# kalakris/stomp_motion_planner_icra2011

Measured on AMD Instinct MI355X. Metric: STOMP iterations/sec (7-DOF, 100 wp, K=512, 256³ SDF) at 1/2/4/8 GPUs, higher is better.
Workload: dtype f64; 1 GPU; cfg2: 7-DOF, 100 wp (N=99), K=512 (512/GPU), K_r=0, 256^3 SDF, S=49 spheres; global_rollouts=512, rollouts_per_gpu=512, parallelism=rollout shard x1

## Files before the change

### stomp_motion_planner_icra2011_amd/csrc/engine.cpp

```cpp
#include "stomp_engine.h"

#include <hip/hip_runtime.h>

#include <algorithm>
#include <chrono>
#include <cmath>
#include <condition_variable>
#include <map>
#include <memory>
#include <mutex>
#include <cstdarg>
#include <cstdio>
#include <cstdlib>
#include <cstring>
#include <string>
#include <thread>
#include <unordered_map>
#include <vector>

#include "kernels.h"
#include "setup.h"

#ifdef STOMP_WITH_RCCL
#include <rccl/rccl.h>
// ... 72 lines not shown
    SetupOutput su;
    DevModel model{};
    TermsModel terms{};
    bool terms_on = false;
    double* d_terms_traj = nullptr;
    uint8_t* d_cs = nullptr;
    DevTrack* d_track = nullptr;
    const int* d_stop = nullptr;
    double* d_opt_costs = nullptr;
    DevTrack* h_track = nullptr;
    bool tracking = false;
    std::vector<FkOp> ops;
    std::vector<int> sphere_slot;
    int nslots = 0;
    std::vector<void*> allocs;
    double *d_theta = nullptr, *d_LT = nullptr, *d_MT = nullptr, *d_QT = nullptr;
    double *d_params = nullptr, *d_noise = nullptr, *d_control = nullptr, *d_prob = nullptr, *d_state = nullptr;
    double *d_params_b = nullptr, *d_noise_b = nullptr, *d_control_b = nullptr, *d_state_b = nullptr;
    int row_set = 0;
    double *d_cum = nullptr, *d_u = nullptr;
    double *d_x_params = nullptr, *d_x_noise = nullptr, *d_x_control = nullptr, *d_x_state = nullptr;
    double *d_last_traj = nullptr, *d_best_traj = nullptr, *d_total = nullptr;
    double *d_pad_pos = nullptr, *d_start = nullptr, *d_goal = nullptr;
    double *d_tot_loc = nullptr, *d_tot_all = nullptr, *d_tot_x = nullptr, *d_slot = nullptr, *d_slot_all = nullptr;
    double* d_reuse_costs = nullptr;
    int* d_reuse_count = nullptr;
    double *d_spec_params = nullptr, *d_spec_noise = nullptr, *d_spec_ctl = nullptr;
    bool spec_on = false;
    bool pick_fuse = true;
    int* d_sel = nullptr;
// ... 319 lines not shown
    const double co0 = cof(1, 1, 2, 2), co1 = cof(1, 2, 2, 0), co2 = cof(1, 0, 2, 1);
    const double det = M[0] * co0 + M[1] * co1 + M[2] * co2;
    const double sc = 1.0 / det;
    O[0] = co0 * sc; O[1] = cof(0, 2, 2, 1) * sc; O[2] = cof(0, 1, 1, 2) * sc;
    O[3] = co1 * sc; O[4] = cof(0, 0, 2, 2) * sc; O[5] = cof(0, 2, 1, 0) * sc;
    O[6] = co2 * sc; O[7] = cof(0, 1, 2, 0) * sc; O[8] = cof(0, 0, 1, 1) * sc;
}

void release(stomp_engine* e)
{
    if (!e) return;
    if (e->stream) hipStreamSynchronize(e->stream);
    for (auto& v : e->evs) { hipEventDestroy(v.a); hipEventDestroy(v.b); }
    for (auto ev : e->pool) hipEventDestroy(ev);
    for (void* p : e->allocs) hipFree(p);
    if (e->h_total) hipHostFree(e->h_total);
    if (e->h_cf) hipHostFree(e->h_cf);
    if (e->h_track) hipHostFree(e->h_track);
    if (e->h_stall) hipHostFree(e->h_stall);
    for (auto& r : e->coll_ring)
        if (r.ev) hipEventDestroy(r.ev);
#ifdef STOMP_WITH_RCCL
    if (e->comm) ncclCommDestroy(e->comm);
#endif
    if (e->ev_ready) hipEventDestroy(e->ev_ready);
    if (e->ev_done) hipEventDestroy(e->ev_done);
    if (e->own_stream && e->stream) hipStreamDestroy(e->stream);
}

void launch_rollouts(stomp_engine* e, const CostArgs& ca)
{
    DevModel& m = e->model;
    const int nro = ca.num_noisy + (ca.x_params ? 1 : 0);
    if (m.lean && m.nsaves > 0 && nro > m.sv_rows) {
        void* q = nullptr;
        if (hipMalloc(&q, sizeof(double) * (size_t)nro * m.nsaves * 12 * m.N) == hipSuccess) {
            e->allocs.push_back(q);
            m.sv_glob = (double*)q;
            m.sv_rows = nro;
        } else {
            (void)hipGetLastError();
            m.lean = 0;
        }
    }
    launch_cost(m, ca, e->stream);
}

void launch_terms_for(stomp_engine* e, const CostArgs& ca, uint8_t* cs = nullptr)
{
    if (!e->terms_on) return;
    Timed tm(e, T_TERMS);
    TermsArgs ta{};
    ta.stop = e->d_stop;
    ta.traj = ca.traj_out; ta.state = ca.state_out; ta.total = ca.total_out; ta.num_noisy = ca.num_noisy;
    ta.cs = cs;
    if (ca.x_params) {
        ta.x_traj = ca.x_traj; ta.x_state = ca.x_state; ta.x_total = ca.x_total; ta.x_cs = e->d_cs;
// ... 949 lines not shown
            int best = per_cu_full;
            for (int lv = 1; lv <= 2; ++lv)
                if (per_cu[lv] > best) {
                    best = per_cu[lv];
                    m.lean = lv;
                }
        }
        if (const char* v = getenv("STOMP_DEBUG_LEAN")) {
            const int lv = atoi(v);
            if (lv >= 0 && lv <= 2 && rollout_lean_allowed(m, lv)) m.lean = lv;
        }
        if (getenv("STOMP_DEBUG_LEAN_PRINT"))
            fprintf(stderr, "stomp: rollout LDS full %zu / lean1 %zu / lean2 %zu B, workgroups per CU %d / %d / %d, "
                            "needed %d, layout lean %d\n", lds, rollout_lds_bytes(m, 0, 1) + stat,
                    rollout_lds_bytes(m, 0, 2) + stat, per_cu[0], per_cu[1], per_cu[2], need, m.lean);
    }
    if (!cost_supported(m)) CREATE_TRY(fail(e, STOMP_E_UNSUPPORTED, "FK program too large (%d ops, %d segments)",
                                            m.nops, m.nseg));
    {
        const RolloutLds L = rollout_lds(J, N, e->S, m.sph_chunk, m.nsaves, m.nseg, m.nops, m.nslots, 1);
        std::vector<unsigned char> img(L.total - L.sph, 0);
        auto put = [&](size_t off, const void* src, size_t bytes) {
            if (bytes) std::memcpy(img.data() + (off - L.sph), src, bytes);
        };
        std::vector<double> jlim(2 * (size_t)J);
        for (int j = 0; j < J; ++j) { jlim[2 * j] = jmin[j]; jlim[2 * j + 1] = jmax[j]; }
        put(L.sph, sph.data(), sizeof(DevSphere) * e->S);
        put(L.seg, segs.data(), sizeof(DevSegment) * segs.size());
        put(L.ops, e->ops.data(), sizeof(FkOp) * e->ops.size());
        put(L.slot, slot_sph.data(), sizeof(int) * slot_sph.size());
// ... 43 lines not shown
    m.ny_d = (double)m.ny; m.nz_d = (double)m.nz;
    m.hi_x = m.nx - 1.5; m.hi_y = m.ny - 1.5; m.hi_z = m.nz - 1.5;
    m.ox = d->grid.origin[0]; m.oy = d->grid.origin[1]; m.oz = d->grid.origin[2]; m.res = d->grid.resolution;
    m.inv_res = 1.0 / d->grid.resolution;
    m.start = e->d_start; m.goal = e->d_goal;
    const double invTime = 1.0 / e->disc;
    for (int k = 0; k < 7; ++k) {
        m.vel_coef[k] = invTime * kDiffRules[0][k];
        if ((k < kVelTap0 || k > kVelTap1) && kDiffRules[0][k] != 0.0)
            CREATE_TRY(fail(e, STOMP_E_UNSUPPORTED, "velocity rule tap %d outside the kernel's stencil", k));
    }
    m.w_obs = e->w_obs; m.w_con = e->w_con; m.w_tq = e->w_tq;
    m.QT = e->d_QT;
    m.split_cap = std::max(e->K_loc + 2, m.cus / 2 + 1);
    CREATE_TRY(dev_alloc(e, &m.split_cnt, (size_t)m.split_cap));
    if (m.lean && m.nsaves > 0) {
        m.sv_rows = e->K_loc + 1;
        CREATE_TRY(dev_alloc(e, &m.sv_glob, (size_t)m.sv_rows * m.nsaves * 12 * N));
    }
    {
        const char* env = std::getenv("STOMP_DEBUG_SPLIT_MAX");
        m.split_max = env ? std::atoi(env) : 0;
        const char* xi = std::getenv("STOMP_DEBUG_XCTL_INLINE");
        m.x_ctl_inline = xi && std::strcmp(xi, "1") == 0 ? 1 : 0;
    }
    if (getenv("STOMP_DEBUG_LEAN_PRINT")) {
        const int nro = e->K_loc + 1, extra = e->pre_on ? e->rows : 0;
        const int P = rollout_split_pieces(m, nro, extra, false);
        const char* body = P ? "split" : nro <= m.cus ? (m.phased_lds > 0 ? "phased" : "wide")
                                                      : (m.lean ? "lean slot loop" : "slot loop");
        fprintf(stderr, "stomp: model J %d N %d S %d nseg %d nops %d nsaves %d sincos_pre %d sph_chunk %d lean %d "
                        "pregen %d fused_noise %d brick %d, launch of %d rollouts: %s, %d pieces\n",
                J, N, e->S, m.nseg, m.nops, m.nsaves, m.sincos_pre, m.sph_chunk, m.lean, e->pre_on ? 1 : 0,
                J <= 16 ? 1 : 0, m.brick, nro, body, P);
    }
    m.pad_collision = 0;
    launch_pad_fk(m, e->d_start, e->d_goal, e->d_pad_pos, e->d_pad_cf, e->stream);
    int pad_cf = 0;
    if (hipMemcpyAsync(&pad_cf, e->d_pad_cf, sizeof(int), hipMemcpyDeviceToHost, e->stream) != hipSuccess ||
        hipStreamSynchronize(e->stream) != hipSuccess)
        CREATE_TRY(fail(e, STOMP_E_DEVICE, "padding FK failed: %s", hipGetErrorString(hipGetLastError())));
    m.pad_collision = pad_cf;
    e->pad_collision = pad_cf;
    if (hipMemcpyAsync(e->d_last_traj, e->d_theta, sizeof(double) * J * N, hipMemcpyDeviceToDevice, e->stream) !=
            hipSuccess ||
        hipMemcpyAsync(e->d_best_traj, e->d_theta, sizeof(double) * J * N, hipMemcpyDeviceToDevice, e->stream) !=
            hipSuccess)
        CREATE_TRY(fail(e, STOMP_E_DEVICE, "trajectory copies failed"));

// ... 1392 lines not shown
```

### stomp_motion_planner_icra2011_amd/csrc/k_cost.hip

```cpp
#include <algorithm>
#include <cassert>
#include <cstdlib>

#include "device_fk.h"
#include "limits_device.h"
#include "noise_device.h"
#include "stamps.h"

namespace stomp {

namespace {
constexpr int kMaxOps = 64;
constexpr int kMaxSeg = 64;
#ifndef ROLLOUT_BLOCK
#define ROLLOUT_BLOCK 256
#endif
constexpr int kBlock = ROLLOUT_BLOCK;
#ifndef ROLLOUT_MIN_WAVES
#define ROLLOUT_MIN_WAVES (ROLLOUT_BLOCK > 256 ? 4 : 3)
#endif
#ifndef ROLLOUT_WIDE_BLOCK
#define ROLLOUT_WIDE_BLOCK 512
#endif
constexpr int kWideBlock = ROLLOUT_WIDE_BLOCK;
// ... 101 lines not shown
    case 10: STOMP_FOLD_STEP(9) [[fallthrough]];
    case 9: STOMP_FOLD_STEP(8) [[fallthrough]];
    case 8: STOMP_FOLD_STEP(7) [[fallthrough]];
    case 7: STOMP_FOLD_STEP(6) [[fallthrough]];
    case 6: STOMP_FOLD_STEP(5) [[fallthrough]];
    case 5: STOMP_FOLD_STEP(4) [[fallthrough]];
    case 4: STOMP_FOLD_STEP(3) [[fallthrough]];
    case 3: STOMP_FOLD_STEP(2) [[fallthrough]];
    case 2: STOMP_FOLD_STEP(1) [[fallthrough]];
    case 1: STOMP_FOLD_STEP(0) break;
    default: break;
    }
#undef STOMP_FOLD_STEP
}

__device__ __forceinline__ double sphere_speed(const DevModel& m, const double* fb, const double* pad,
                                               const DevSphere& sp, int s, int t)
{
    const int N = m.N;
    double y[7][3];
#pragma unroll
    for (int kk = kVelTap0; kk <= kVelTap1; ++kk) {
        const int tt = t + kk - 3;
        double yf[3];
        apply_lds(fb, N, min(max(tt, 0), N - 1), sp.pos, yf);
        const int row = tt < 0 ? tt + 6 : (tt >= N ? tt - N + 6 : 0);
        const double* src = pad + (row * m.S + s) * 3;
        const bool in = tt >= 0 && tt < N;
#pragma unroll
        for (int c = 0; c < 3; ++c) y[kk][c] = in ? yf[c] : src[c];
    }
    double v0 = 0.0, v1 = 0.0, v2 = 0.0;
#pragma unroll
    for (int kk = kVelTap0; kk <= kVelTap1; ++kk) {
        const double c = m.vel_coef[kk];
        if (c == 0.0) continue;
        v0 += c * y[kk][0];
        v1 += c * y[kk][1];
        v2 += c * y[kk][2];
    }
    return sqrt(v0 * v0 + v1 * v1 + v2 * v2);
}

// ... 113 lines not shown
        for (int u = 0; u < 4; ++u) v[u] = a.x_params[min(idx0 + tid + u * BLOCK, J * N - 1)];
#pragma unroll
        for (int u = 0; u < 4; ++u) {
            const int idx = idx0 + tid + u * BLOCK;
            if (idx < J * N) {
                a.x_prm[idx] = v[u];
                a.x_nse[idx] = 0.0;
                const int d = idx / N, i = idx - d * N;
                zA[d * Nall + i + 6] = v[u] + 0.0;
            }
        }
    }
    rollout_control<BLOCK>(a.nz, 0, zA, zB, tid, a.x_ctl);
}

template <int BLOCK, bool BRICK, bool PHASED = false, bool FK_OVERLAP = true, int LEAN = 0>
__device__ __forceinline__ void rollout_body(const DevModel& m, const CostArgs& a, const int bid)
{
    static_assert(!LEAN || (!PHASED && FK_OVERLAP), "the lean layout is the slot loop's");
    extern __shared__ __attribute__((aligned(16))) unsigned char lds_raw[];
    __shared__ int flag;
    __shared__ int nz_count;
    const int J = m.J, N = m.N, S = m.S;
    const RolloutLds L = rollout_lds(J, N, S, m.sph_chunk, m.nsaves, m.nseg, m.nops, m.nslots, LEAN ? 0 : m.pad_lds,
                                     PHASED, LEAN);
    {
        const int nro = a.num_noisy + (a.x_params ? 1 : 0);
        if (bid >= nro) {
            const int r = bid - nro;
            if (r >= a.pre_rows) {
                totals_block<BLOCK>(a, J, N, r - a.pre_rows, (double*)(lds_raw + L.nzA));
                return;
            }
            const bool own = PHASED && r >= a.row0 && r < a.row0 + a.num_noisy;
            pregen_block<BLOCK>(a, r, own, (double*)(lds_raw + L.nzA), (double*)(lds_raw + L.nzB));
            return;
        }
    }
    if (a.pre_rows > 0 || a.tot_rows > 0) __builtin_amdgcn_s_setprio(2);
    if (a.stop && *a.stop) return;
    double* traj = (double*)(lds_raw + L.traj);
    double* fb = (double*)(lds_raw + L.fb);
    double* sv = LEAN ? global_ptr(m.sv_glob) + (size_t)bid * m.nsaves * 12 * N : (double*)(lds_raw + L.sv);
    double* av = (double*)(lds_raw + L.av);
    unsigned short* nzl = (unsigned short*)(lds_raw + L.nzl);
    const unsigned char* gimg = (const unsigned char*)m.img;
    const DevSphere* sph = (const DevSphere*)(lds_raw + L.sph);
    const DevSegment* seg_s = (const DevSegment*)(lds_raw + L.seg);
    const FkOp* ops_s = (const FkOp*)(lds_raw + L.ops);
    const int* hl_s = (const int*)(lds_raw + L.hl);
    const double* jlim_s = (const double*)(lds_raw + L.jlim);
    CSphere* csph = (CSphere*)gimg;
    CSegment* cseg = (CSegment*)(gimg + (L.seg - L.sph));
    COp* cops = (COp*)(gimg + (L.ops - L.sph));
    CInt* chl = (CInt*)(gimg + (L.hl - L.sph));
    CDouble* cjlim = (CDouble*)(gimg + (L.jlim - L.sph));
    auto op_at = [&](int i) -> FkOp {
        if constexpr (LEAN != 0) return load_op(cops + i);
        else return ops_s[i];
    };
    const double* pad = !LEAN && m.pad_lds ? (const double*)(lds_raw + L.pad) : m.pad_pos;
    const bool sincos_pre = !LEAN && m.sincos_pre;

    STAMP(0);
    BLOCK_BEGIN();
    const int e = bid, tid = threadIdx.x, lane = tid & 63, wv = tid >> 6;
    constexpr int NW = BLOCK / 64;
    const bool extra = e == a.num_noisy;
    const int member = extra ? a.x_member : a.member;
    double* zA = (double*)(lds_raw + L.nzA);
    double* zB = (double*)(lds_raw + L.nzB);
    const bool gen = a.fused_noise == 1 && !extra;
    const bool pre = a.fused_noise == 2 && !extra;
    constexpr int kCopyBatch = 12 * 256 / BLOCK;
    unsigned long long img[kCopyBatch];
    const int nw = LEAN == 0 ? m.img_words : LEAN == 1 ? (int)(S * sizeof(DevSphere) / 8) : 0;
    if constexpr (LEAN != 2) {
#pragma unroll
        for (int u = 0; u < kCopyBatch; ++u) img[u] = m.img[min(tid + u * BLOCK, nw - 1)];
    }
    PreChunk pc0;
    const bool priced = !PHASED && a.ctl_by_pre;
    const int pr = e + a.row0;
    if (pre) {
        if (priced) pre_chunk_load<BLOCK, false>(a.nz, pr, 0, tid, pc0);
        else pre_chunk_load<BLOCK>(a.nz, pr, 0, tid, pc0);
    }
    if (gen) {
        rollout_normals<BLOCK>(a.nz, e, zA, zB, tid);
    } else if (!pre) {
        const double* prm = extra ? a.x_params : a.params + (long long)e * a.stride;
// ... 30 lines not shown
    if (gen) {
        if (defer) rollout_project<BLOCK, true>(a.nz, e, traj, zA, zB, tid);
        else rollout_project<BLOCK>(a.nz, e, traj, zA, zB, tid);
    } else if (pre) {
        if (priced) rollout_from_pre<BLOCK, true, false>(a.nz, pr, e == 0, traj, zA, zB, tid, pc0);
        else if (defer) rollout_from_pre<BLOCK, true>(a.nz, pr, e == 0, traj, zA, zB, tid, pc0);
        else rollout_from_pre<BLOCK>(a.nz, pr, e == 0, traj, zA, zB, tid, pc0);
    }
    if (tid == 0) flag = 0;
    __syncthreads();
    STAMP(1);
    BLOCK_MARK(4);

    {
        __builtin_amdgcn_s_setprio(3);
        if constexpr (LEAN != 0) joint_limit_passes<NW>(m, traj, chl, cjlim, lane, wv);
        else joint_limit_passes<NW>(m, traj, hl_s, jlim_s, lane, wv);
        __builtin_amdgcn_s_setprio(2);
        __syncthreads();
    }
    STAMP(2);
    BLOCK_MARK(5);
    double* tout = extra ? a.x_traj : (a.traj_out ? a.traj_out + (long long)e * J * N : nullptr);
    if (tout)
        for (int idx = tid; idx < J * N; idx += BLOCK) tout[idx] = traj[idx];
    __syncthreads();
    STAMP(3);

    const int t_own = tid - ((N <= 128 && (e & 1)) ? 128 : 0);
    const bool fk_lane = t_own >= 0 && t_own < N;
    const int G = BLOCK / N, pg = tid / N, pt = tid - pg * N;
    Frame C;
    double cum = 0.0, state = 0.0;
    bool col = false;
    auto fk_step = [&](const FkOp& o, const DevSegment& sg) {
        double st = 0.0, ct = 1.0;
        if (sg.q_index >= 0) {
            if (sincos_pre) {
                st = traj[sg.q_index * N + t_own];
                ct = sv[sg.q_index * N + t_own];
            } else {
                det_sincos(traj[sg.q_index * N + t_own], &st, &ct);
            }
        }
        Frame nf;
        if (o.base == kBaseChain) {
            compose(sg, &C, st, ct, nf);
        } else if (o.base == kBaseRoot) {
            compose(sg, nullptr, st, ct, nf);
        } else {
            Frame pf;
            const double* src = sv + (size_t)o.base * 12 * N + t_own;
#pragma unroll
            for (int k = 0; k < 9; ++k) pf.R[k] = src[k * N];
#pragma unroll
            for (int k = 0; k < 3; ++k) pf.p[k] = src[(9 + k) * N];
            compose(sg, &pf, st, ct, nf);
        }
        C = nf;
        if (o.save >= 0) {
            double* dst = sv + (size_t)o.save * 12 * N + t_own;
#pragma unroll
            for (int k = 0; k < 9; ++k) dst[k * N] = C.R[k];
#pragma unroll
            for (int k = 0; k < 3; ++k) dst[(9 + k) * N] = C.p[k];
        }
    };
    auto fk_op = [&](const FkOp& o) {
        if (o.seg < 0 || !fk_lane) return;
        if constexpr (LEAN != 0) {
            const DevSegment sg = load_seg(cseg + o.seg);
            fk_step(o, sg);
        } else {
            fk_step(o, seg_s[o.seg]);
        }
    };
    auto fk_advance = [&](int op) -> int {
        for (; op < m.nops; ++op) {
            const FkOp o = op_at(op);
            fk_op(o);
            if (o.sph_end > o.sph_begin) return op;
        }
        return m.nops;
    };
    if (sincos_pre) {
        const int JN = J * N;
        for (int i0 = tid; i0 - tid < JN; i0 += 3 * BLOCK) {
            double q[3], sn[3], cs[3];
#pragma unroll
            for (int u = 0; u < 3; ++u) q[u] = traj[min(i0 + u * BLOCK, JN - 1)];
#pragma unroll
            for (int u = 0; u < 3; ++u) det_sincos(q[u], &sn[u], &cs[u]);
#pragma unroll
            for (int u = 0; u < 3; ++u) {
                if (i0 + u * BLOCK < JN) {
                    traj[i0 + u * BLOCK] = sn[u];
                    sv[i0 + u * BLOCK] = cs[u];
                }
            }
        }
        __syncthreads();
    }
    if constexpr (PHASED) {
        __builtin_amdgcn_s_setprio(3);
        const int fk_off = t_own - tid;
        const int fk_w0 = -fk_off / 64, fk_w1 = (N - 1 - fk_off) / 64;
        static_assert(!PHASED || BLOCK >= 512, "the phased body prices rows on its non-FK waves");
        if (defer && (wv < fk_w0 || wv > fk_w1)) {
            const int nfk = fk_w1 - fk_w0 + 1;
            const int cw = wv < fk_w0 ? wv : wv - nfk;
            for (int d = cw; d < J; d += NW - nfk)
                wave_control(a.nz, (size_t)pr * J * N, zA, zB, d, lane);
// ... 67 lines not shown
        __syncthreads();
        STAMP(11);
        __builtin_amdgcn_s_setprio(3);
        for (int i = tid; i < nz_count; i += BLOCK) {
            const int it = nzl[i];
            const int qi = it / N, ti = it - qi * N;
            const DevSphere& sp = sph[qi];
            const double pot = potential(sp, sdf_metres(m, (unsigned)av[it]));
            av[it] = pot * sphere_speed(m, fb + (size_t)sp.slot * 12 * N, pad, sp, qi, ti);
        }
        __syncthreads();
        STAMP(12);
        if (fk_lane) fold_avalues(av + t_own, N, S, cum, state);
        __builtin_amdgcn_s_setprio(2);
        STAMP(13);
    } else {
    __builtin_amdgcn_s_setprio(3);
    int op = fk_advance(0);
    __builtin_amdgcn_s_setprio(2);
    int run = 0;
    STAMP(7);
    while (op < m.nops) {
        const FkOp o = op_at(op);
        if (fk_lane) {
#pragma unroll
            for (int k = 0; k < 9; ++k) fb[k * N + t_own] = C.R[k];
#pragma unroll
            for (int k = 0; k < 3; ++k) fb[(9 + k) * N + t_own] = C.p[k];
        }
        if (tid == 0) nz_count = 0;
// ... 25 lines not shown
                    x[i] = F[3 * i] * pos[0] + F[3 * i + 1] * pos[1] + F[3 * i + 2] * pos[2] + F[9 + i];
                bool ok;
                const unsigned idx = sdf_cell<BRICK>(m, x, ok);
                dv[u] = m.sdf[idx];
                okm |= (unsigned)ok << u;
            }
        }
        STAMP(40 + run);
        int next_op = op;
        if constexpr (FK_OVERLAP) {
            __builtin_amdgcn_s_setprio(3);
            next_op = fk_advance(op + 1);
            __builtin_amdgcn_s_setprio(2);
        }
        if (pg < G) {
#pragma unroll
            for (int u = 0; u < kLaneSpheres; ++u) {
                if (u * G >= ns) break;
                const int q = LEAN == 2 ? u : pg + u * G;
                const bool in = q < ns;
                bool nz = false;
                if (in) {
                    int zl, cl;
                    if constexpr (LEAN == 2) {
                        zl = csph[sb + q].zero_lim;
                        cl = csph[sb + q].col_lim;
                    } else {
                        zl = sph[sb + q].zero_lim;
                        cl = sph[sb + q].col_lim;
                    }
                    const int d2 = (okm >> u) & 1u ? (int)dv[u] : 0;
                    col |= d2 < cl;
                    nz = d2 < zl;
                    av[q * N + pt] = nz ? (double)d2 : 0.0;
                }
                const unsigned long long mask = __ballot(nz);
                if (mask) {
                    const int lane_id = tid & 63;
                    const int leader = __ffsll((long long)mask) - 1;
                    int base = 0;
                    if (lane_id == leader) base = atomicAdd(&nz_count, __popcll(mask));
                    base = __shfl(base, leader, 64);
                    if (nz) nzl[base + __popcll(mask & ((1ull << lane_id) - 1ull))] = (unsigned short)(q * N + pt);
                }
            }
        }
        __syncthreads();
        STAMP(11 + 4 * run);
        __builtin_amdgcn_s_setprio(3);
        for (int i = tid; i < nz_count; i += BLOCK) {
            const int it = nzl[i];
            const int qi = it / N, ti = it - qi * N;
            if constexpr (LEAN == 2) {
                const DevSphere sp = load_sph(csph + sb + qi);
                const double pot = potential(sp, sdf_metres(m, (unsigned)av[it]));
                av[it] = pot * sphere_speed(m, fb, pad, sp, sb + qi, ti);
            } else {
                const DevSphere& sp = sph[sb + qi];
// ... 43 lines not shown
            for (; k + 8 <= N; k += 8) {
                double v[8];
#pragma unroll
                for (int q = 0; q < 8; ++q) v[q] = av[k + q];
#pragma unroll
                for (int q = 0; q < 8; ++q) s += v[q];
            }
            for (; k < N; ++k) s += av[k];
            *to = s;
        }
    }
    STAMP(5);
    BLOCK_END();
}

template <int BLOCK, bool BRICK, int LEAN = 0>
__global__ __launch_bounds__(BLOCK, rollout_min_waves<BLOCK>()) void k_rollout(DevModel m, CostArgs a)
{
    rollout_body<BLOCK, BRICK, false, true, LEAN>(m, a, blockIdx.x);
}

template <bool BRICK>
__global__ __launch_bounds__(kWideBlock, kWideBlock > 512 ? 4 : 2) void k_rollout_phased(DevModel m, CostArgs a)
{
    rollout_body<kWideBlock, BRICK, true>(m, a, blockIdx.x);
}

template <int BLOCK, bool BRICK>
__global__ __launch_bounds__(BLOCK, rollout_min_waves<BLOCK>()) void k_rollout_group(const DevModel* ms, const CostArgs* as,
                                                                           int engines, int nro, int npre)
{
    const int b = blockIdx.x;
    int p, bid;
    if (b < engines * nro) {
// ... 464 lines not shown
}

void launch_cost_group(const DevModel& m0, const DevModel* ms, const CostArgs* as, int engines, int nro, int npre,
                       hipStream_t s)
{
    if (engines * (nro + npre) <= 0) return;
    if (m0.brick) launch_cost_group_t<true>(m0, ms, as, engines, nro, npre, s);
    else launch_cost_group_t<false>(m0, ms, as, engines, nro, npre, s);
}

bool cost_supported(const DevModel& m)
{
    return m.nops <= kMaxOps && m.nseg <= kMaxSeg && m.nslots <= kMaxSeg && m.J <= kMaxJoints && m.N <= kBlock;
}

size_t rollout_lds_bytes(const DevModel& m, int pad_lds, int lean)
{
    return rollout_lds(m.J, m.N, m.S, m.sph_chunk, m.nsaves, m.nseg, m.nops, m.nslots, lean ? 0 : pad_lds, false,
                       lean).total;
}

size_t rollout_phased_lds_bytes(const DevModel& m)
{
    const size_t dyn = rollout_lds(m.J, m.N, m.S, m.sph_chunk, m.nsaves, m.nseg, m.nops, m.nslots, m.pad_lds, true).total;
    hipFuncAttributes attr;
    size_t stat = 2048;
    if (hipFuncGetAttributes(&attr, (const void*)k_rollout_phased<false>) == hipSuccess) stat = attr.sharedSizeBytes;
    if ((size_t)m.S * m.N > 65535 || dyn + stat > kLdsPerCu) return 0;
    return dyn;
}

size_t rollout_static_lds()
{
    hipFuncAttributes attr;
    if (hipFuncGetAttributes(&attr, (const void*)k_rollout<kBlock, false>) != hipSuccess) return 2048;
    return attr.sharedSizeBytes;
}

bool rollout_lean_allowed(const DevModel& m, int lean)
{
    return lean == 0 || lean == 1 || (lean == 2 && m.N > kBlock / 2 && m.N <= kBlock);
}

int rollout_blocks_per_cu(size_t lds_total, int lean)
{
    hipFuncAttributes attr;
    int regs = 256;
    const void* fn = lean == 2 ? (const void*)k_rollout<kBlock, false, 2>
                   : lean == 1 ? (const void*)k_rollout<kBlock, false, 1> : (const void*)k_rollout<kBlock, false>;
    if (hipFuncGetAttributes(&attr, fn) == hipSuccess && attr.numRegs > 0)
        regs = attr.numRegs;
    const int alloc = (regs + 7) / 8 * 8;
    int waves_per_simd = 512 / alloc;
    if (waves_per_simd > 8) waves_per_simd = 8;
    const int by_regs = waves_per_simd * 4 / (kBlock / 64);
    const int by_lds = (int)(kLdsPerCu / (lds_total ? lds_total : 1));
    return by_regs < by_lds ? by_regs : by_lds;
}

template <bool BRICK>
static void launch_cost_t(const DevModel& m, const CostArgs& a, hipStream_t s)
{
    const int nro = a.num_noisy + (a.x_params ? 1 : 0);
// ... 12 lines not shown
                           dim3(kSplitBlock), ls, s, m, b);
        return;
    }
    assert(a.spec_rows == 0);
    if (kWideBlock != kBlock && nro <= m.cus && m.phased_lds > 0) {
        const size_t lp = m.phased_lds;
        lds_opt_in((const void*)k_rollout_phased<BRICK>, lp);
        hipLaunchKernelGGL(k_rollout_phased<BRICK>, dim3(blocks), dim3(kWideBlock), lp, s, m, a);
        return;
    }
    if (kWideBlock != kBlock && nro <= m.cus) {
        if (lds > 64 * 1024) lds_opt_in((const void*)k_rollout<kWideBlock, BRICK>, lds);
        hipLaunchKernelGGL((k_rollout<kWideBlock, BRICK>), dim3(blocks), dim3(kWideBlock), lds, s, m, a);
        return;
    }
    if (m.lean) {
        assert(nro <= m.sv_rows || m.nsaves == 0);
        const size_t ll = rollout_lds_bytes(m, 0, m.lean);
        if (m.lean == 2) {
            if (ll > 64 * 1024) lds_opt_in((const void*)k_rollout<kBlock, BRICK, 2>, ll);
            hipLaunchKernelGGL((k_rollout<kBlock, BRICK, 2>), dim3(blocks), dim3(kBlock), ll, s, m, a);
        } else {
            if (ll > 64 * 1024) lds_opt_in((const void*)k_rollout<kBlock, BRICK, 1>, ll);
            hipLaunchKernelGGL((k_rollout<kBlock, BRICK, 1>), dim3(blocks), dim3(kBlock), ll, s, m, a);
        }
        return;
    }
    if (lds > 64 * 1024) lds_opt_in((const void*)k_rollout<kBlock, BRICK>, lds);
    hipLaunchKernelGGL((k_rollout<kBlock, BRICK>), dim3(blocks), dim3(kBlock), lds, s, m, a);
}
// ... 11 lines not shown
```

### stomp_motion_planner_icra2011_amd/csrc/kernels.h

```cpp
#pragma once

#include <hip/hip_runtime.h>
#include <stdint.h>

namespace stomp {

constexpr int kMaxJoints = 32;
constexpr int kRunMaxSmall = 16;
constexpr int kRunMaxLarge = 8;
constexpr int kSaves = 2;
constexpr int kSumBlock = 64;
constexpr int kBandBatch = 8;
constexpr int kMatPadRows = 16 * kBandBatch;
constexpr int kVelTap0 = 2;
constexpr int kVelTap1 = 5;
constexpr int kNoiseJT = 4;

inline int run_max(int N) { return N <= 128 ? kRunMaxSmall : kRunMaxLarge; }

constexpr int kBaseChain = -2;
constexpr int kBaseRoot = -1;

struct DevSegment {
    int parent, q_index;
    int rot_identity, pad_;
    double rot[9];
    double trans[3];
    double axis[3];
};

// ... 31 lines not shown
    double ny_d, nz_d;
    double hi_x, hi_y, hi_z;
    const double* start;
    const double* goal;
    double vel_coef[7];
    double w_obs, w_con, w_tq;
    int pad_collision;
    const double* QT;
    int* split_cnt;
    int split_cap;
    int split_max;
    int x_ctl_inline;
    int lean;
    double* sv_glob;
    int sv_rows;
};


struct RolloutLds {
    size_t traj, fb, sv, av, nzl, nzA, nzB, sph, seg, ops, slot, hl, jlim, pad, total;
};


__host__ __device__ inline size_t align16(size_t x) { return (x + 15) & ~(size_t)15; }

__host__ __device__ inline int noise_jp(int J) { return (J + kNoiseJT - 1) / kNoiseJT * kNoiseJT; }

__host__ __device__ inline RolloutLds rollout_lds(int J, int N, int S, int max_slot, int nsaves, int nseg, int nops,
                                                  int nslots, int pad_lds, bool phased = false, int lean = 0)
{
    RolloutLds l;
    if (phased) max_slot = S;
    l.traj = 0;
    l.fb = l.traj + (size_t)J * N * sizeof(double);
    l.sv = l.fb + (size_t)(phased ? nslots : 1) * 12 * N * sizeof(double);
    l.av = l.sv + (size_t)(lean ? 0 : nsaves) * 12 * N * sizeof(double);
    l.nzl = l.av + (size_t)max_slot * N * sizeof(double);
    const size_t nzw = (size_t)(N + kBandBatch) * noise_jp(J) > (size_t)J * (N + 12)
                           ? (size_t)(N + kBandBatch) * noise_jp(J) : (size_t)J * (N + 12);
    l.nzA = l.fb;
    if (phased && (size_t)S * N * (sizeof(double) + sizeof(unsigned short)) >= 2 * nzw * sizeof(double)) l.nzA = l.av;
    l.nzB = l.nzA + nzw * sizeof(double);
    size_t end = l.nzl + (size_t)max_slot * N * sizeof(unsigned short);
    if (l.nzB + nzw * sizeof(double) > end) end = l.nzB + nzw * sizeof(double);
    l.sph = align16(end);
    l.seg = align16(l.sph + (size_t)S * sizeof(DevSphere));
    l.ops = align16(l.seg + (size_t)nseg * sizeof(DevSegment));
    l.slot = align16(l.ops + (size_t)nops * sizeof(FkOp));
    l.hl = align16(l.slot + (size_t)(nslots + 1) * sizeof(int));
    l.jlim = align16(l.hl + (size_t)J * sizeof(int));
    l.pad = align16(l.jlim + (size_t)2 * J * sizeof(double));
    l.total = l.pad + (pad_lds ? (size_t)36 * S * sizeof(double) : 0);
    if (lean) {
        l.total = lean == 1 ? l.seg : l.sph;
    }
    return l;
}

struct Sigma {
    double v[kMaxJoints];
};

struct NoiseArgs {
    int J, N, Nall, K_loc, first_global, K_gen_global, iteration;
    uint64_t seed;
    Sigma sigma;
    const double* theta;
    const double* LT;
    const double* MT;
// ... 142 lines not shown
                         hipStream_t s);
size_t price_candidate_lds_bytes(int J, int N);
void launch_pregen(const NoiseArgs& a, int rows, hipStream_t s);

struct DevTrack {
    int stop, cfi, iterations, success, success_iteration, collision_success_iteration, last_improvement_iteration;
    int pad;
    double best;
    unsigned long long t0, t_success, t_collision_success;
};
void launch_track_start(DevTrack* tr, hipStream_t s);
void launch_track(DevTrack* tr, int it, int max_it_cf, const double* total, const uint8_t* cf, const uint8_t* cs,
                  double* costs, const double* last_traj, double* best_traj, int JN, hipStream_t s);
void launch_cost(const DevModel& m, const CostArgs& a, hipStream_t s);
bool cost_supported(const DevModel& m);
size_t rollout_lds_bytes(const DevModel& m, int pad_lds, int lean = 0);
size_t rollout_phased_lds_bytes(const DevModel& m);
size_t rollout_static_lds();
int rollout_blocks_per_cu(size_t lds_total, int lean = 0);
bool rollout_lean_allowed(const DevModel& m, int lean);
constexpr size_t kLdsPerCu = 144 * 1024;
constexpr size_t kRolloutLdsMax = 156 * 1024;
void launch_cumulative(const WeightArgs& a, double* cum, hipStream_t s);
void launch_weights(const WeightArgs& a, hipStream_t s);
int weights_tile(int K_loc);
void launch_update(int J, int N, const double* MT, const double* u, const double* u_all, int nb_total,
                   double* theta, const int* stop, hipStream_t s, double* delta = nullptr);
struct UpdateArgs {
    const double* MT;
    const double* u;
    double* theta;
    const int* stop;
};
void launch_cost_group(const DevModel& m0, const DevModel* ms, const CostArgs* as, int engines, int nro, int npre,
// ... 59 lines not shown
```

Before: 17270 iterations/s.

## Add opt-in look-ahead rollout layout overlapping next FK with SDF lookups

```diff
diff --git a/stomp_motion_planner_icra2011_amd/csrc/engine.cpp b/stomp_motion_planner_icra2011_amd/csrc/engine.cpp
--- a/stomp_motion_planner_icra2011_amd/csrc/engine.cpp
+++ b/stomp_motion_planner_icra2011_amd/csrc/engine.cpp
@@ -110,6 +110,11 @@
     std::vector<int> sphere_slot;
     int nslots = 0;
     std::vector<void*> allocs;
+    struct Retired {
+        void* p;
+        hipEvent_t ev;
+    };
+    std::vector<Retired> sv_retired;
     double *d_theta = nullptr, *d_LT = nullptr, *d_MT = nullptr, *d_QT = nullptr;
     double *d_params = nullptr, *d_noise = nullptr, *d_control = nullptr, *d_prob = nullptr, *d_state = nullptr;
     double *d_params_b = nullptr, *d_noise_b = nullptr, *d_control_b = nullptr, *d_state_b = nullptr;
@@ -459,6 +464,7 @@
     for (auto& v : e->evs) { hipEventDestroy(v.a); hipEventDestroy(v.b); }
     for (auto ev : e->pool) hipEventDestroy(ev);
     for (void* p : e->allocs) hipFree(p);
+    for (auto& r : e->sv_retired) { hipFree(r.p); hipEventDestroy(r.ev); }
     if (e->h_total) hipHostFree(e->h_total);
     if (e->h_cf) hipHostFree(e->h_cf);
     if (e->h_track) hipHostFree(e->h_track);
@@ -477,15 +483,50 @@
 {
     DevModel& m = e->model;
     const int nro = ca.num_noisy + (ca.x_params ? 1 : 0);
-    if (m.lean && m.nsaves > 0 && nro > m.sv_rows) {
+    for (size_t i = 0; i < e->sv_retired.size();) {
+        if (hipEventQuery(e->sv_retired[i].ev) == hipSuccess) {
+            hipFree(e->sv_retired[i].p);
+            hipEventDestroy(e->sv_retired[i].ev);
+            e->sv_retired.erase(e->sv_retired.begin() + i);
+        } else {
+            (void)hipGetLastError();
+            ++i;
+        }
+    }
+    if ((m.lean || m.lookahead) && m.nsaves > 0 && nro > m.sv_rows) {
+        const size_t row = sizeof(double) * (size_t)m.nsaves * 12 * m.N;
+        int rows = std::max(nro, 2 * m.sv_rows);
         void* q = nullptr;
-        if (hipMalloc(&q, sizeof(double) * (size_t)nro * m.nsaves * 12 * m.N) == hipSuccess) {
+        if (hipMalloc(&q, row * rows) != hipSuccess) {
+            (void)hipGetLastError();
+            rows = nro;
+            if (hipMalloc(&q, row * rows) != hipSuccess) {
+                (void)hipGetLastError();
+                q = nullptr;
+            }
+        }
+        hipEvent_t ev = nullptr;
+        if (q && (hipEventCreateWithFlags(&ev, hipEventDisableTiming) != hipSuccess ||
+                  hipEventRecord(ev, e->stream) != hipSuccess)) {
+            (void)hipGetLastError();
+            if (ev) hipEventDestroy(ev);
+            hipFree(q);
+            q = nullptr;
+        }
+        if (q) {
+            auto it = std::find(e->allocs.begin(), e->allocs.end(), (void*)m.sv_glob);
+            if (it != e->allocs.end()) {
+                e->allocs.erase(it);
+                e->sv_retired.push_back({(void*)m.sv_glob, ev});
+            } else {
+                hipEventDestroy(ev);
+            }
             e->allocs.push_back(q);
             m.sv_glob = (double*)q;
-            m.sv_rows = nro;
+            m.sv_rows = rows;
         } else {
-            (void)hipGetLastError();
             m.lean = 0;
+            m.lookahead = 0;
         }
     }
     launch_cost(m, ca, e->stream);
@@ -1465,6 +1506,21 @@
             fprintf(stderr, "stomp: rollout LDS full %zu / lean1 %zu / lean2 %zu B, workgroups per CU %d / %d / %d, "
                             "needed %d, layout lean %d\n", lds, rollout_lds_bytes(m, 0, 1) + stat,
                     rollout_lds_bytes(m, 0, 2) + stat, per_cu[0], per_cu[1], per_cu[2], need, m.lean);
+        m.lookahead = 0;
+        const bool slot_loop = e->K_loc + 1 > cus;
+        size_t la_lds[3] = {0, 0, 0};
+        int la_per_cu[3] = {0, 0, 0};
+        for (int lv = 1; lv <= 2; ++lv) {
+            la_lds[lv] = rollout_lds_bytes(m, 0, 0, lv == 1 && m.sincos_pre ? 2 : 1) + stat;
+            if (slot_loop && la_lds[lv] <= kRolloutLdsMax) la_per_cu[lv] = rollout_blocks_per_cu(la_lds[lv], 0, 1);
+        }
+        if (const char* v = getenv("STOMP_DEBUG_LOOKAHEAD")) {
+            const int lv = atoi(v);
+            if (lv >= 1 && lv <= 2 && la_per_cu[lv] >= 1) m.lookahead = lv;
+        }
+        if (getenv("STOMP_DEBUG_LEAN_PRINT"))
+            fprintf(stderr, "stomp: rollout LDS look-ahead %zu / without the pre-pass %zu B, workgroups per CU %d / %d, "
+                            "layout look-ahead %d\n", la_lds[1], la_lds[2], la_per_cu[1], la_per_cu[2], m.lookahead);
     }
     if (!cost_supported(m)) CREATE_TRY(fail(e, STOMP_E_UNSUPPORTED, "FK program too large (%d ops, %d segments)",
                                             m.nops, m.nseg));
@@ -1538,7 +1594,7 @@
     m.QT = e->d_QT;
     m.split_cap = std::max(e->K_loc + 2, m.cus / 2 + 1);
     CREATE_TRY(dev_alloc(e, &m.split_cnt, (size_t)m.split_cap));
-    if (m.lean && m.nsaves > 0) {
+    if ((m.lean || m.lookahead) && m.nsaves > 0) {
         m.sv_rows = e->K_loc + 1;
         CREATE_TRY(dev_alloc(e, &m.sv_glob, (size_t)m.sv_rows * m.nsaves * 12 * N));
     }
@@ -1554,9 +1610,9 @@
         const char* body = P ? "split" : nro <= m.cus ? (m.phased_lds > 0 ? "phased" : "wide")
                                                       : (m.lean ? "lean slot loop" : "slot loop");
         fprintf(stderr, "stomp: model J %d N %d S %d nseg %d nops %d nsaves %d sincos_pre %d sph_chunk %d lean %d "
-                        "pregen %d fused_noise %d brick %d, launch of %d rollouts: %s, %d pieces\n",
+                        "pregen %d fused_noise %d brick %d, launch of %d rollouts: %s, %d pieces, lookahead %d\n",
                 J, N, e->S, m.nseg, m.nops, m.nsaves, m.sincos_pre, m.sph_chunk, m.lean, e->pre_on ? 1 : 0,
-                J <= 16 ? 1 : 0, m.brick, nro, body, P);
+                J <= 16 ? 1 : 0, m.brick, nro, body, P, m.lookahead);
     }
     m.pad_collision = 0;
     launch_pad_fk(m, e->d_start, e->d_goal, e->d_pad_pos, e->d_pad_cf, e->stream);
diff --git a/stomp_motion_planner_icra2011_amd/csrc/k_cost.hip b/stomp_motion_planner_icra2011_amd/csrc/k_cost.hip
--- a/stomp_motion_planner_icra2011_amd/csrc/k_cost.hip
+++ b/stomp_motion_planner_icra2011_amd/csrc/k_cost.hip
@@ -139,8 +139,9 @@
 #undef STOMP_FOLD_STEP
 }
 
+template <bool STAGED = false>
 __device__ __forceinline__ double sphere_speed(const DevModel& m, const double* fb, const double* pad,
-                                               const DevSphere& sp, int s, int t)
+                                               const DevSphere& sp, int s, int t, int ps = 0)
 {
     const int N = m.N;
     double y[7][3];
@@ -150,8 +151,8 @@
         double yf[3];
         apply_lds(fb, N, min(max(tt, 0), N - 1), sp.pos, yf);
         const int row = tt < 0 ? tt + 6 : (tt >= N ? tt - N + 6 : 0);
-        const double* src = pad + (row * m.S + s) * 3;
         const bool in = tt >= 0 && tt < N;
+        const double* src = STAGED ? pad + ((in ? 0 : row - kVelPadRow0) * ps + s) * 3 : pad + (row * m.S + s) * 3;
 #pragma unroll
         for (int c = 0; c < 3; ++c) y[kk][c] = in ? yf[c] : src[c];
     }
@@ -295,16 +296,18 @@
     rollout_control<BLOCK>(a.nz, 0, zA, zB, tid, a.x_ctl);
 }
 
-template <int BLOCK, bool BRICK, bool PHASED = false, bool FK_OVERLAP = true, int LEAN = 0>
+template <int BLOCK, bool BRICK, bool PHASED = false, bool FK_OVERLAP = true, int LEAN = 0, bool LA = false>
 __device__ __forceinline__ void rollout_body(const DevModel& m, const CostArgs& a, const int bid)
 {
     static_assert(!LEAN || (!PHASED && FK_OVERLAP), "the lean layout is the slot loop's");
+    static_assert(!LA || (!LEAN && !PHASED && FK_OVERLAP), "the look-ahead layout is the slot loop's, in place of lean");
+    constexpr bool CT = LEAN != 0 || LA;
     extern __shared__ __attribute__((aligned(16))) unsigned char lds_raw[];
     __shared__ int flag;
     __shared__ int nz_count;
     const int J = m.J, N = m.N, S = m.S;
-    const RolloutLds L = rollout_lds(J, N, S, m.sph_chunk, m.nsaves, m.nseg, m.nops, m.nslots, LEAN ? 0 : m.pad_lds,
-                                     PHASED, LEAN);
+    const RolloutLds L = rollout_lds(J, N, S, m.sph_chunk, m.nsaves, m.nseg, m.nops, m.nslots, CT ? 0 : m.pad_lds,
+                                     PHASED, LEAN, LA ? lookahead_layout(m) : 0);
     {
         const int nro = a.num_noisy + (a.x_params ? 1 : 0);
         if (bid >= nro) {
@@ -322,13 +325,15 @@
     if (a.stop && *a.stop) return;
     double* traj = (double*)(lds_raw + L.traj);
     double* fb = (double*)(lds_raw + L.fb);
-    double* sv = LEAN ? global_ptr(m.sv_glob) + (size_t)bid * m.nsaves * 12 * N : (double*)(lds_raw + L.sv);
+    double* sv = CT ? global_ptr(m.sv_glob) + (size_t)bid * m.nsaves * 12 * N : (double*)(lds_raw + L.sv);
     double* av = (double*)(lds_raw + L.av);
     unsigned short* nzl = (unsigned short*)(lds_raw + L.nzl);
     const unsigned char* gimg = (const unsigned char*)m.img;
     const DevSphere* sph = (const DevSphere*)(lds_raw + L.sph);
     const DevSegment* seg_s = (const DevSegment*)(lds_raw + L.seg);
     const FkOp* ops_s = (const FkOp*)(lds_raw + L.ops);
+    double* pst = (double*)(lds_raw + L.pst);
+    double* csn = (double*)(lds_raw + L.cs);
     const int* hl_s = (const int*)(lds_raw + L.hl);
     const double* jlim_s = (const double*)(lds_raw + L.jlim);
     CSphere* csph = (CSphere*)gimg;
@@ -337,11 +342,11 @@
     CInt* chl = (CInt*)(gimg + (L.hl - L.sph));
     CDouble* cjlim = (CDouble*)(gimg + (L.jlim - L.sph));
     auto op_at = [&](int i) -> FkOp {
-        if constexpr (LEAN != 0) return load_op(cops + i);
+        if constexpr (CT) return load_op(cops + i);
         else return ops_s[i];
     };
-    const double* pad = !LEAN && m.pad_lds ? (const double*)(lds_raw + L.pad) : m.pad_pos;
-    const bool sincos_pre = !LEAN && m.sincos_pre;
+    const double* pad = !CT && m.pad_lds ? (const double*)(lds_raw + L.pad) : m.pad_pos;
+    const bool sincos_pre = LA ? m.sincos_pre && m.lookahead == 1 : !LEAN && m.sincos_pre;
 
     STAMP(0);
     BLOCK_BEGIN();
@@ -355,7 +360,7 @@
     const bool pre = a.fused_noise == 2 && !extra;
     constexpr int kCopyBatch = 12 * 256 / BLOCK;
     unsigned long long img[kCopyBatch];
-    const int nw = LEAN == 0 ? m.img_words : LEAN == 1 ? (int)(S * sizeof(DevSphere) / 8) : 0;
+    const int nw = !CT ? m.img_words : LEAN != 2 ? (int)(S * sizeof(DevSphere) / 8) : 0;
     if constexpr (LEAN != 2) {
 #pragma unroll
         for (int u = 0; u < kCopyBatch; ++u) img[u] = m.img[min(tid + u * BLOCK, nw - 1)];
@@ -416,7 +421,7 @@
 
     {
         __builtin_amdgcn_s_setprio(3);
-        if constexpr (LEAN != 0) joint_limit_passes<NW>(m, traj, chl, cjlim, lane, wv);
+        if constexpr (CT) joint_limit_passes<NW>(m, traj, chl, cjlim, lane, wv);
         else joint_limit_passes<NW>(m, traj, hl_s, jlim_s, lane, wv);
         __builtin_amdgcn_s_setprio(2);
         __syncthreads();
@@ -440,7 +445,7 @@
         if (sg.q_index >= 0) {
             if (sincos_pre) {
                 st = traj[sg.q_index * N + t_own];
-                ct = sv[sg.q_index * N + t_own];
+                ct = csn[sg.q_index * N + t_own];
             } else {
                 det_sincos(traj[sg.q_index * N + t_own], &st, &ct);
             }
@@ -470,7 +475,7 @@
     };
     auto fk_op = [&](const FkOp& o) {
         if (o.seg < 0 || !fk_lane) return;
-        if constexpr (LEAN != 0) {
+        if constexpr (CT) {
             const DevSegment sg = load_seg(cseg + o.seg);
             fk_step(o, sg);
         } else {
@@ -497,7 +502,7 @@
             for (int u = 0; u < 3; ++u) {
                 if (i0 + u * BLOCK < JN) {
                     traj[i0 + u * BLOCK] = sn[u];
-                    sv[i0 + u * BLOCK] = cs[u];
+                    csn[i0 + u * BLOCK] = cs[u];
                 }
             }
         }
@@ -595,6 +600,153 @@
         if (fk_lane) fold_avalues(av + t_own, N, S, cum, state);
         __builtin_amdgcn_s_setprio(2);
         STAMP(13);
+    } else if constexpr (LA) {
+    auto publish = [&](int b) {
+        if (fk_lane) {
+            double* dst = fb + (size_t)b * 12 * N + t_own;
+#pragma unroll
+            for (int k = 0; k < 9; ++k) dst[k * N] = C.R[k];
+#pragma unroll
+            for (int k = 0; k < 3; ++k) dst[(9 + k) * N] = C.p[k];
+        }
+    };
+    auto fk_advance_la = [&](int op, bool& moved) -> int {
+        moved = false;
+        for (; op < m.nops; ++op) {
+            const FkOp o = op_at(op);
+            fk_op(o);
+            moved |= o.seg >= 0;
+            if (o.sph_end > o.sph_begin) return op;
+        }
+        return m.nops;
+    };
+    unsigned dv[kLaneSpheres];
+    unsigned okm = 0;
+    auto lookups = [&](const double* f, int sb, int ns) {
+        okm = 0;
+        double F[12];
+#pragma unroll
+        for (int k = 0; k < 12; ++k) F[k] = f[k * N + pt];
+#pragma unroll
+        for (int u = 0; u < kLaneSpheres; ++u) {
+            if (u * G >= ns) break;
+            const double* ps = sph[sb + min(pg + u * G, ns - 1)].pos;
+            double pos[3];
+#pragma unroll
+            for (int i = 0; i < 3; ++i) pos[i] = ps[i];
+            double x[3];
+#pragma unroll
+            for (int i = 0; i < 3; ++i)
+                x[i] = F[3 * i] * pos[0] + F[3 * i + 1] * pos[1] + F[3 * i + 2] * pos[2] + F[9 + i];
+            bool ok;
+            const unsigned idx = sdf_cell<BRICK>(m, x, ok);
+            dv[u] = m.sdf[idx];
+            okm |= (unsigned)ok << u;
+        }
+    };
+    static_assert(kVelPadRows * 3 * kRunMaxSmall <= BLOCK, "one staged padding position per lane");
+    auto stage_load = [&](int sb, int ns) -> double {
+        const int l = min(tid, kVelPadRows * 3 * ns - 1), r3 = l / (3 * ns);
+        return pad[((kVelPadRow0 + r3) * S + sb) * 3 + (l - r3 * 3 * ns)];
+    };
+    auto stage_store = [&](int ns, double v) {
+        if (tid < kVelPadRows * 3 * ns) pst[tid] = v;
+    };
+    __builtin_amdgcn_s_setprio(3);
+    int op = fk_advance(0);
+    __builtin_amdgcn_s_setprio(2);
+    int run = 0;
+    STAMP(7);
+    if (op < m.nops) {
+        FkOp o = op_at(op);
+        double pv = stage_load(o.sph_begin, o.sph_end - o.sph_begin);
+        publish(0);
+        stage_store(o.sph_end - o.sph_begin, pv);
+        if (tid == 0) nz_count = 0;
+        __syncthreads();
+        lookups(fb, o.sph_begin, o.sph_end - o.sph_begin);
+        STAMP(40);
+        bool moved;
+        __builtin_amdgcn_s_setprio(3);
+        int op1 = fk_advance_la(op + 1, moved);
+        int cur = 0, nxt = moved ? 1 : 0;
+        if (op1 < m.nops && moved) publish(1);
+        __builtin_amdgcn_s_setprio(2);
+        for (;;) {
+            const int sb = o.sph_begin, ns = o.sph_end - sb;
+            STAMP(10 + 4 * run);
+            if (pg < G) {
+#pragma unroll
+                for (int u = 0; u < kLaneSpheres; ++u) {
+                    if (u * G >= ns) break;
+                    const int q = pg + u * G;
+                    const bool in = q < ns;
+                    bool nz = false;
+                    if (in) {
+                        const int zl = sph[sb + q].zero_lim, cl = sph[sb + q].col_lim;
+                        const int d2 = (okm >> u) & 1u ? (int)dv[u] : 0;
+                        col |= d2 < cl;
+                        nz = d2 < zl;
+                        av[q * N + pt] = nz ? (double)d2 : 0.0;
+                    }
+                    const unsigned long long mask = __ballot(nz);
+                    if (mask) {
+                        const int lane_id = tid & 63;
+                        const int leader = __ffsll((long long)mask) - 1;
+                        int base = 0;
+                        if (lane_id == leader) base = atomicAdd(&nz_count, __popcll(mask));
+                        base = __shfl(base, leader, 64);
+                        if (nz) nzl[base + __popcll(mask & ((1ull << lane_id) - 1ull))] = (unsigned short)(q * N + pt);
+                    }
+                }
+            }
+            __syncthreads();
+            STAMP(11 + 4 * run);
+            const bool more = op1 < m.nops;
+            FkOp o1 = o;
+            if (more) {
+                o1 = op_at(op1);
+                pv = stage_load(o1.sph_begin, o1.sph_end - o1.sph_begin);
+                lookups(fb + (size_t)nxt * 12 * N, o1.sph_begin, o1.sph_end - o1.sph_begin);
+            }
+            STAMP(40 + run + 1);
+            __builtin_amdgcn_s_setprio(3);
+            const double* fbr = fb + (size_t)cur * 12 * N;
+            for (int i = tid; i < nz_count; i += BLOCK) {
+                const int it = nzl[i];
+                const int qi = it / N, ti = it - qi * N;
+                const DevSphere& sp = sph[sb + qi];
+                const double pot = potential(sp, sdf_metres(m, (unsigned)av[it]));
+                av[it] = pot * sphere_speed<true>(m, fbr, pst, sp, qi, ti, ns);
+            }
+            __syncthreads();
+            STAMP(12 + 4 * run);
+            if (more && fk_lane) {
+                const double* src = fb + (size_t)nxt * 12 * N + t_own;
+#pragma unroll
+                for (int k = 0; k < 9; ++k) C.R[k] = src[k * N];
+#pragma unroll
+                for (int k = 0; k < 3; ++k) C.p[k] = src[(9 + k) * N];
+            }
+            if (fk_lane) fold_avalues(av + t_own, N, ns, cum, state);
+            if (!more) break;
+            const int op2 = fk_advance_la(op1 + 1, moved);
+            const int b2 = moved ? nxt ^ 1 : nxt;
+            if (op2 < m.nops && moved) publish(b2);
+            stage_store(o1.sph_end - o1.sph_begin, pv);
+            if (tid == 0) nz_count = 0;
+            __builtin_amdgcn_s_setprio(2);
+            STAMP(13 + 4 * run);
+            __syncthreads();
+            cur = nxt;
+            nxt = b2;
+            op1 = op2;
+            o = o1;
+            ++run;
+        }
+        __builtin_amdgcn_s_setprio(2);
+        STAMP(13 + 4 * run);
+    }
     } else {
     __builtin_amdgcn_s_setprio(3);
     int op = fk_advance(0);
@@ -650,6 +802,8 @@
             __builtin_amdgcn_s_setprio(2);
         }
         if (pg < G) {
+            unsigned nzm = 0;
+            int wave_pairs = 0;
 #pragma unroll
             for (int u = 0; u < kLaneSpheres; ++u) {
                 if (u * G >= ns) break;
@@ -670,14 +824,23 @@
                     nz = d2 < zl;
                     av[q * N + pt] = nz ? (double)d2 : 0.0;
                 }
-                const unsigned long long mask = __ballot(nz);
-                if (mask) {
-                    const int lane_id = tid & 63;
-                    const int leader = __ffsll((long long)mask) - 1;
-                    int base = 0;
-                    if (lane_id == leader) base = atomicAdd(&nz_count, __popcll(mask));
-                    base = __shfl(base, leader, 64);
+                nzm |= (unsigned)nz << u;
+                wave_pairs += __popcll(__ballot(nz));
+            }
+            if (wave_pairs) {
+                const int lane_id = tid & 63;
+                const int leader = __ffsll((long long)__ballot(true)) - 1;
+                int base = 0;
+                if (lane_id == leader) base = atomicAdd(&nz_count, wave_pairs);
+                base = __shfl(base, leader, 64);
+#pragma unroll
+                for (int u = 0; u < kLaneSpheres; ++u) {
+                    if (u * G >= ns) break;
+                    const bool nz = (nzm >> u) & 1u;
+                    const unsigned long long mask = __ballot(nz);
+                    const int q = LEAN == 2 ? u : pg + u * G;
                     if (nz) nzl[base + __popcll(mask & ((1ull << lane_id) - 1ull))] = (unsigned short)(q * N + pt);
+                    base += __popcll(mask);
                 }
             }
         }
@@ -751,10 +914,10 @@
     BLOCK_END();
 }
 
-template <int BLOCK, bool BRICK, int LEAN = 0>
+template <int BLOCK, bool BRICK, int LEAN = 0, bool LA = false>
 __global__ __launch_bounds__(BLOCK, rollout_min_waves<BLOCK>()) void k_rollout(DevModel m, CostArgs a)
 {
-    rollout_body<BLOCK, BRICK, false, true, LEAN>(m, a, blockIdx.x);
+    rollout_body<BLOCK, BRICK, false, true, LEAN, LA>(m, a, blockIdx.x);
 }
 
 template <bool BRICK>
@@ -1249,10 +1412,11 @@
     return m.nops <= kMaxOps && m.nseg <= kMaxSeg && m.nslots <= kMaxSeg && m.J <= kMaxJoints && m.N <= kBlock;
 }
 
-size_t rollout_lds_bytes(const DevModel& m, int pad_lds, int lean)
-{
-    return rollout_lds(m.J, m.N, m.S, m.sph_chunk, m.nsaves, m.nseg, m.nops, m.nslots, lean ? 0 : pad_lds, false,
-                       lean).total;
+size_t rollout_lds_bytes(const DevModel& m, int pad_lds, int lean, int lookahead)
+{
+    if (lookahead) lean = 0;
+    return rollout_lds(m.J, m.N, m.S, m.sph_chunk, m.nsaves, m.nseg, m.nops, m.nslots, lean || lookahead ? 0 : pad_lds,
+                       false, lean, lookahead).total;
 }
 
 size_t rollout_phased_lds_bytes(const DevModel& m)
@@ -1277,11 +1441,12 @@
     return lean == 0 || lean == 1 || (lean == 2 && m.N > kBlock / 2 && m.N <= kBlock);
 }
 
-int rollout_blocks_per_cu(size_t lds_total, int lean)
+int rollout_blocks_per_cu(size_t lds_total, int lean, int lookahead)
 {
     hipFuncAttributes attr;
     int regs = 256;
-    const void* fn = lean == 2 ? (const void*)k_rollout<kBlock, false, 2>
+    const void* fn = lookahead ? (const void*)k_rollout<kBlock, false, 0, true>
+                   : lean == 2 ? (const void*)k_rollout<kBlock, false, 2>
                    : lean == 1 ? (const void*)k_rollout<kBlock, false, 1> : (const void*)k_rollout<kBlock, false>;
     if (hipFuncGetAttributes(&attr, fn) == hipSuccess && attr.numRegs > 0)
         regs = attr.numRegs;
@@ -1324,6 +1489,13 @@
         hipLaunchKernelGGL((k_rollout<kWideBlock, BRICK>), dim3(blocks), dim3(kWideBlock), lds, s, m, a);
         return;
     }
+    if (m.lookahead) {
+        assert(nro <= m.sv_rows || m.nsaves == 0);
+        const size_t ll = rollout_lds_bytes(m, 0, 0, lookahead_layout(m));
+        if (ll > 64 * 1024) lds_opt_in((const void*)k_rollout<kBlock, BRICK, 0, true>, ll);
+        hipLaunchKernelGGL((k_rollout<kBlock, BRICK, 0, true>), dim3(blocks), dim3(kBlock), ll, s, m, a);
+        return;
+    }
     if (m.lean) {
         assert(nro <= m.sv_rows || m.nsaves == 0);
         const size_t ll = rollout_lds_bytes(m, 0, m.lean);
diff --git a/stomp_motion_planner_icra2011_amd/csrc/kernels.h b/stomp_motion_planner_icra2011_amd/csrc/kernels.h
--- a/stomp_motion_planner_icra2011_amd/csrc/kernels.h
+++ b/stomp_motion_planner_icra2011_amd/csrc/kernels.h
@@ -14,6 +14,7 @@
 constexpr int kMatPadRows = 16 * kBandBatch;
 constexpr int kVelTap0 = 2;
 constexpr int kVelTap1 = 5;
+constexpr int kVelPadRows = kVelTap1 - kVelTap0, kVelPadRow0 = kVelTap0 + 3;
 constexpr int kNoiseJT = 4;
 
 inline int run_max(int N) { return N <= 128 ? kRunMaxSmall : kRunMaxLarge; }
@@ -75,11 +76,17 @@
     int lean;
     double* sv_glob;
     int sv_rows;
-};
+    int lookahead;
+};
+
+__host__ __device__ inline int lookahead_layout(const DevModel& m)
+{
+    return !m.lookahead ? 0 : (m.lookahead == 1 && m.sincos_pre ? 2 : 1);
+}
 
 
 struct RolloutLds {
-    size_t traj, fb, sv, av, nzl, nzA, nzB, sph, seg, ops, slot, hl, jlim, pad, total;
+    size_t traj, fb, sv, cs, av, pst, nzl, nzA, nzB, sph, seg, ops, slot, hl, jlim, pad, total;
 };
 
 
@@ -88,15 +95,19 @@
 __host__ __device__ inline int noise_jp(int J) { return (J + kNoiseJT - 1) / kNoiseJT * kNoiseJT; }
 
 __host__ __device__ inline RolloutLds rollout_lds(int J, int N, int S, int max_slot, int nsaves, int nseg, int nops,
-                                                  int nslots, int pad_lds, bool phased = false, int lean = 0)
+                                                  int nslots, int pad_lds, bool phased = false, int lean = 0,
+                                                  int lookahead = 0)
 {
     RolloutLds l;
     if (phased) max_slot = S;
     l.traj = 0;
     l.fb = l.traj + (size_t)J * N * sizeof(double);
-    l.sv = l.fb + (size_t)(phased ? nslots : 1) * 12 * N * sizeof(double);
-    l.av = l.sv + (size_t)(lean ? 0 : nsaves) * 12 * N * sizeof(double);
-    l.nzl = l.av + (size_t)max_slot * N * sizeof(double);
+    l.sv = l.fb + (size_t)(phased ? nslots : lookahead ? 2 : 1) * 12 * N * sizeof(double);
+    l.cs = l.sv;
+    l.av = l.sv + (lookahead ? (size_t)(lookahead == 2 ? J : 0) * N * sizeof(double)
+                             : (size_t)(lean ? 0 : nsaves) * 12 * N * sizeof(double));
+    l.pst = l.av + (size_t)max_slot * N * sizeof(double);
+    l.nzl = l.pst + (lookahead ? (size_t)kVelPadRows * max_slot * 3 * sizeof(double) : 0);
     const size_t nzw = (size_t)(N + kBandBatch) * noise_jp(J) > (size_t)J * (N + 12)
                            ? (size_t)(N + kBandBatch) * noise_jp(J) : (size_t)J * (N + 12);
     l.nzA = l.fb;
@@ -112,8 +123,8 @@
     l.jlim = align16(l.hl + (size_t)J * sizeof(int));
     l.pad = align16(l.jlim + (size_t)2 * J * sizeof(double));
     l.total = l.pad + (pad_lds ? (size_t)36 * S * sizeof(double) : 0);
-    if (lean) {
-        l.total = lean == 1 ? l.seg : l.sph;
+    if (lean || lookahead) {
+        l.total = lean == 2 ? l.sph : l.seg;
     }
     return l;
 }
@@ -286,10 +297,10 @@
                   double* costs, const double* last_traj, double* best_traj, int JN, hipStream_t s);
 void launch_cost(const DevModel& m, const CostArgs& a, hipStream_t s);
 bool cost_supported(const DevModel& m);
-size_t rollout_lds_bytes(const DevModel& m, int pad_lds, int lean = 0);
+size_t rollout_lds_bytes(const DevModel& m, int pad_lds, int lean = 0, int lookahead = 0);
 size_t rollout_phased_lds_bytes(const DevModel& m);
 size_t rollout_static_lds();
-int rollout_blocks_per_cu(size_t lds_total, int lean = 0);
+int rollout_blocks_per_cu(size_t lds_total, int lean = 0, int lookahead = 0);
 bool rollout_lean_allowed(const DevModel& m, int lean);
 constexpr size_t kLdsPerCu = 144 * 1024;
 constexpr size_t kRolloutLdsMax = 156 * 1024;
```

Result: no change. 17150 iterations/s (-0.7%).
